# simonsobs/pixell

Measured on AMD Instinct MI355X. Metric: map2alm+alm2map round-trips/sec, higher is better.
Workload: dtype f64

## Files before the change

pixell_amd/csrc/leg_s0.hip:

```cpp
#include "legendre_dev.hpp"

namespace pxs {

#define S0_PHASE_A \
	while (k + 4 <= nk) { \
		bool act = false; \
		_Pragma("unroll") for (int s = 0; s < K; s++) act |= LEG_IS_LIVE(lam2[s], sc[s]); \
		if (__any(act)) break; \
		const double4_t q0 = LDC(coef, k), q1 = LDC(coef, k+1), q2 = LDC(coef, k+2), q3 = LDC(coef, k+3); \
		const double b0 = polar ? q0.c : q0.b, b1 = polar ? q1.c : q1.b, b2 = polar ? q2.c : q2.b, b3 = polar ? q3.c : q3.b; \
		_Pragma("unroll") for (int s = 0; s < K; s++) { \
			lam1[s] = fma(fma(q0.a, csq[s], b0), lam2[s], lam1[s]); \
			lam2[s] = fma(fma(q1.a, csq[s], b1), lam1[s], lam2[s]); \
			lam1[s] = fma(fma(q2.a, csq[s], b2), lam2[s], lam1[s]); \
			lam2[s] = fma(fma(q3.a, csq[s], b3), lam1[s], lam2[s]); \
			if (sc[s] < 0 && fabs(lam2[s]) > SC_BIG) { lam1[s] *= SC_SMALL; lam2[s] *= SC_SMALL; sc[s]++; } \
		} \
		k += 4; \
	}
#define S0_SEEDED_PHASE_A \
	if (a.seed_mode == 2) { \
		const double* sd = a.seed_d + ((long)m*a.nwave + wv)*(2*K*64); const int* si = a.seed_i + ((long)m*a.nwave + wv)*((K+1)*64); \
		k = PXS_UNIFORM_INT(si[K*64]); \
		_Pragma("unroll") for (int s = 0; s < K; s++) { lam1[s] = sd[s*64 + lane]; lam2[s] = sd[(K+s)*64 + lane]; sc[s] = si[s*64 + lane]; } \
	} else { \
		S0_PHASE_A \
		if (a.seed_mode == 1) { \
			double* sd = a.seed_d + ((long)m*a.nwave + wv)*(2*K*64); int* si = a.seed_i + ((long)m*a.nwave + wv)*((K+1)*64); \
			_Pragma("unroll") for (int s = 0; s < K; s++) { sd[s*64 + lane] = lam1[s]; sd[(K+s)*64 + lane] = lam2[s]; si[s*64 + lane] = sc[s]; } \
			if (lane == 0) si[K*64] = k; \
		} \
	}

#define S0_SYN_PAIR(c0, c1, a0, a1) { \
	PXS_VCOPY(vb0, polar ? c0.c : c0.b); \
	PXS_VCOPY(vb1, polar ? c1.c : c1.b); \
	_Pragma("unroll") for (int s = 0; s < K; s++) { \
		p1r[s] = fma(lam2[s], a0.a, p1r[s]); p1i[s] = fma(lam2[s], a0.b, p1i[s]); \
		p2r[s] = fma(lam2[s], a0.c, p2r[s]); p2i[s] = fma(lam2[s], a0.d, p2i[s]); \
		lam1[s] = fma(fma(c0.a, csq[s], vb0), lam2[s], lam1[s]); \
	} \
	_Pragma("unroll") for (int s = 0; s < K; s++) { \
		p1r[s] = fma(lam1[s], a1.a, p1r[s]); p1i[s] = fma(lam1[s], a1.b, p1i[s]); \
		p2r[s] = fma(lam1[s], a1.c, p2r[s]); p2i[s] = fma(lam1[s], a1.d, p2i[s]); \
		lam2[s] = fma(fma(c1.a, csq[s], vb1), lam1[s], lam2[s]); \
	} }

template<int K> __global__ __launch_bounds__(64, (K == 4 ? 7 : 1)) void leg_syn_s0(const LegK a)
{
	const int lane = threadIdx.x; int wv, m, bb;
	if (!leg_block(a, wv, m, bb)) return;
	const long row0 = PXS_UNIFORM_LONG(a.row[m]);
	const int nk = (a.lmax - m)/2 + 1;
	const double4_t* __restrict__ coef = a.coef + row0;
	const double4_t* __restrict__ at = reinterpret_cast<const double4_t*>(a.almt + (long)bb*a.almt_bs) + row0;
	double x[K], csq[K], lam1[K], lam2[K], p1r[K], p1i[K], p2r[K], p2i[K];
	int sc[K], rn[K], rs[K];
	bool alive_any = false;
	const bool polar = leg_wave_polar(a, wv, K);
#pragma unroll
	for (int s = 0; s < K; s++) {
		const int p = leg_pair_u(a, wv, K, s, lane);
		const bool valid = leg_pair_valid(a, p);
		rn[s] = valid ? a.ring_n[p] : -1; rs[s] = valid ? a.ring_s[p] : -1;
		x[s] = valid ? a.cth[p] : 0.0;
		const double sth = valid ? a.sth[p] : 0.0;
		csq[s] = polar ? -sth*sth : x[s]*x[s];
		const bool alive = valid && ((double)m <= a.lmax*sth + a.ofs);
		lam1[s] = 0; lam2[s] = 0; sc[s] = 0;
		if (alive && a.seed_mode != 2) { double mt; int e; pow_scaled(sth, m, mt, e); to_scaled(mt, e, lam2[s], sc[s]); }
		p1r[s] = p1i[s] = p2r[s] = p2i[s] = 0;
		alive_any |= alive;
	}
	int k = 0;
	if (__any(alive_any)) {
		S0_SEEDED_PHASE_A
		k = PXS_UNIFORM_INT(k); coef = (const double4_t*)PXS_UNIFORM_LONG((long)coef);
		PXS_COUNT(0, (long)(nk - k)*K*6 + (a.seed_mode != 2 ? (long)k*K*2 : 0L));
		while (k + 1 < nk) {
			bool pend = false;
#pragma unroll
			for (int s = 0; s < K; s++) pend |= (sc[s] < 0);
			if (!__any(pend)) break;
			for (int it = 0; it < 2 && k + 1 < nk; it++, k += 2) {
				const double4_t c0 = LDC(coef, k), c1 = LDC(coef, k+1), a0 = LDC(at, k), a1 = LDC(at, k+1);
				S0_SYN_PAIR(c0, c1, a0, a1)
			}
#pragma unroll
			for (int s = 0; s < K; s++)
				if (sc[s] < 0 && fabs(lam2[s]) > SC_BIG) {
					lam1[s] *= SC_SMALL; lam2[s] *= SC_SMALL;
					if (++sc[s] == 0) p1r[s] = p1i[s] = p2r[s] = p2i[s] = 0;
				}
		}
#pragma unroll
		for (int s = 0; s < K; s++) if (sc[s] < 0) { p1r[s] = p1i[s] = p2r[s] = p2i[s] = 0; lam1[s] = lam2[s] = 0; }
		double4_t c0 = LDC(coef, k), c1 = LDC(coef, k+1), a0 = LDC(at, k), a1 = LDC(at, k+1);
		while (k + 3 < nk) {
			double4_t n0 = LDC(coef, k+2), n1 = LDC(coef, k+3), m0 = LDC(at, k+2), m1 = LDC(at, k+3);
			S0_SYN_PAIR(c0, c1, a0, a1)
			k += 2;
			c0 = LDC(coef, k+2); c1 = LDC(coef, k+3); a0 = LDC(at, k+2); a1 = LDC(at, k+3);
			S0_SYN_PAIR(n0, n1, m0, m1)
			k += 2;
		}
		for (; k + 1 < nk; k += 2) {
			const double4_t n0 = LDC(coef, k+2), n1 = LDC(coef, k+3), m0 = LDC(at, k+2), m1 = LDC(at, k+3);
			S0_SYN_PAIR(c0, c1, a0, a1)
			c0 = n0; c1 = n1; a0 = m0; a1 = m1;
		}
		if (k < nk) {
#pragma unroll
			for (int s = 0; s < K; s++) {
				p1r[s] = fma(lam2[s], a0.a, p1r[s]); p1i[s] = fma(lam2[s], a0.b, p1i[s]);
				p2r[s] = fma(lam2[s], a0.c, p2r[s]); p2i[s] = fma(lam2[s], a0.d, p2i[s]);
			}
		}
	}
	double2* __restrict__ out = a.leg + (long)bb*a.leg_bs + (long)m*a.ld;
#pragma unroll
	for (int s = 0; s < K; s++) {
		const int p = leg_pair_u(a, wv, K, s, lane);
		const bool valid = leg_pair_valid(a, p);
		const int rn_ = valid ? a.ring_n[p] : -1, rs_ = valid ? a.ring_s[p] : -1;
		const double x_ = valid ? a.cth[p] : 0.0;
		if (rn_ >= 0) out[rn_] = make_double2(p1r[s] + x_*p2r[s], p1i[s] + x_*p2i[s]);
		if (rs_ >= 0) out[rs_] = make_double2(p1r[s] - x_*p2r[s], p1i[s] - x_*p2i[s]);
	}
}

#define S0_ANA_PAIR(c0, c1) { \
	PXS_VCOPY(vb0, polar ? c0.c : c0.b); \
	PXS_VCOPY(vb1, polar ? c1.c : c1.b); \
	double t0 = 0, t1 = 0, t2 = 0, t3 = 0, u0 = 0, u1 = 0, u2 = 0, u3 = 0; \
	_Pragma("unroll") for (int s = 0; s < K; s++) { \
		t0 = fma(lam2[s], d1r[s], t0); t1 = fma(lam2[s], d1i[s], t1); t2 = fma(lam2[s], d2r[s], t2); t3 = fma(lam2[s], d2i[s], t3); \
		lam1[s] = fma(fma(c0.a, csq[s], vb0), lam2[s], lam1[s]); \
	} \
	_Pragma("unroll") for (int s = 0; s < K; s++) { \
		u0 = fma(lam1[s], d1r[s], u0); u1 = fma(lam1[s], d1i[s], u1); u2 = fma(lam1[s], d2r[s], u2); u3 = fma(lam1[s], d2i[s], u3); \
		lam2[s] = fma(fma(c1.a, csq[s], vb1), lam1[s], lam2[s]); \
	} \
	 \
	LEG_RED_PUT(kk, t0, t1, t2, t3) \
	LEG_RED_PUT(kk+1, u0, u1, u2, u3) \
	kk += 2; \
	if (kk == LEG_FSTEPS) { leg_flush(red, pout + 4*kbase, lane, LEG_FSTEPS, a.atomic); kk = 0; kbase = k+2; } }

template<int K> __global__ __launch_bounds__(64) void leg_ana_s0(const LegK a)
{
	PXS_SHARED(double, red);
	const int lane = threadIdx.x; int wv, m, bb;
	if (!leg_block(a, wv, m, bb)) return;
	const long row0 = PXS_UNIFORM_LONG(a.row[m]);
	const int nk = (a.lmax - m)/2 + 1;
	const double4_t* __restrict__ coef = a.coef + row0;
	double* __restrict__ pout = a.part + (long)bb*a.mom_bs + ((long)wv*a.rows_chunk + (row0 - a.rowbase))*4;
	const double2* __restrict__ in = a.leg + (long)bb*a.leg_bs + (long)m*a.ld;
	double csq[K], lam1[K], lam2[K], d1r[K], d1i[K], d2r[K], d2i[K];
	int sc[K];
	bool alive_any = false;
	const bool polar = leg_wave_polar(a, wv, K);
	auto load_data = [&](int s) {
// ... 163 lines not shown
```

pixell_amd/csrc/legendre.hip:

```cpp
#include "legendre_dev.hpp"
#include <thread>
#include <memory>
#include <functional>
#include <string>

namespace pxs {

static constexpr int K_SYN0 = 4, K_ANA0 = 8, K_SYNS = 3, K_ANAS = 4;

__device__ __forceinline__ double2 ld_alm(const void* alm, int dtype, long idx) {
	if (dtype == PX_C64) { float2 v = ((const float2*)alm)[idx]; return make_double2(v.x, v.y); }
	return ((const double2*)alm)[idx];
}
__device__ __forceinline__ void st_alm(void* alm, int dtype, long idx, double2 v) {
	if (dtype == PX_C64) ((float2*)alm)[idx] = make_float2((float)v.x, (float)v.y);
	else ((double2*)alm)[idx] = v;
}
__device__ __forceinline__ double eps_lm(int l, int m) {
	if (l <= m) return 0.0;
	double L = l, M = m;
	return sqrt((L*L - M*M)/(4.0*L*L - 1.0));
}

struct AlmK {
// ... 95 lines not shown
		o[2] = -sg*be[u]*(e.x + b.y); o[3] = -sg*be[u]*(e.y - b.x);
	}
}
__global__ __launch_bounds__(256) void alm_post_spin(AlmK a) {
	const int m = blockIdx.y;
	const int l0 = max(m, a.spin);
	const int lb = blockIdx.x*(256*ALM_U) + threadIdx.x + min(m, l0);
	if (lb > a.lmax) return;
	const long base = (long)a.mstart[m], row = a.row[m];
	void* alm = alm_of_batch(a);
	double M0[ALM_U], M1[ALM_U], M2[ALM_U], M3[ALM_U], be[ALM_U];
#pragma unroll
	for (int u = 0; u < ALM_U; u++) {
		const int l = lb + 256*u;
		const bool ok = l <= a.lmax && l >= l0;
		const long r = row + (l - l0);
		const double* M = a.mom + (long)blockIdx.z*a.mom_bs + 4*r;
		M0[u] = ok ? M[0] : 0.0; M1[u] = ok ? M[1] : 0.0; M2[u] = ok ? M[2] : 0.0; M3[u] = ok ? M[3] : 0.0;
		be[u] = ok ? a.alpha[r] : 0.0;
	}
	const double sg = (a.spin & 1) ? -1.0 : 1.0;
#pragma unroll
	for (int u = 0; u < ALM_U; u++) {
		const int l = lb + 256*u;
		if (l > a.lmax) break;
		const long idx = base + (long)l*a.lstride;
		const double2 E = make_double2(-0.5*be[u]*(M0[u] + sg*M2[u]), -0.5*be[u]*(M1[u] + sg*M3[u]));
		const double2 B = make_double2(-0.5*be[u]*(M1[u] - sg*M3[u]),  0.5*be[u]*(M0[u] - sg*M2[u]));
		if (a.deriv1) { const double f = sqrt((double)l*(l+1.0)); st_alm(alm, a.dtype, idx, make_double2(f*E.x, f*E.y)); }
		else { st_alm(alm, a.dtype, idx, E); st_alm(alm, a.dtype, idx + a.cstride, B); }
	}
}

__global__ __launch_bounds__(256) void reduce_partials(const double* __restrict__ part, double* __restrict__ mom, const long* __restrict__ row,
		const int* __restrict__ first, int m0, int nmc, long rowbase, long rows_chunk, int nwave)
{
	const int mi = blockIdx.y;
	const long r0 = row[m0 + mi], nrow = row[m0 + mi + 1] - r0;
	const long i = (long)blockIdx.x*blockDim.x + threadIdx.x;
	if (i >= 4*nrow) return;
	const int step = (int)(i >> 2);
	const long off = (r0 - rowbase)*4 + i;
	double s = 0;
	for (int w = 0; w < nwave; w++) {
		const int f = first[w*nmc + mi];
		if (f > 0 && step >= f - 1) s += part[(long)w*rows_chunk*4 + off];
	}
	mom[r0*4 + i] = s;
}

__global__ __launch_bounds__(256) void coef2_kernel(const double4_t* __restrict__ coef, long nrows, double2* __restrict__ c2, double2* __restrict__ c2p) {
	const long i = (long)blockIdx.x*blockDim.x + threadIdx.x;
	if (i >= nrows + 32) return;
	if (i < nrows) { const double4_t c = coef[i]; c2[i] = make_double2(c.a, c.b); c2p[i] = make_double2(c.a, c.c); }
	else { c2[i] = make_double2(0, 0); c2p[i] = make_double2(0, 0); }
}


void LegProfile::begin(hipStream_t st, int stage) {
	if (!enabled) return;
	hipEvent_t e; PXS_HIP(hipEventCreate(&e)); PXS_HIP(hipEventRecord(e, st)); open_.push_back(e);
}
void LegProfile::end(hipStream_t st, int stage) {
	if (!enabled || open_.empty()) return;
	hipEvent_t e; PXS_HIP(hipEventCreate(&e)); PXS_HIP(hipEventRecord(e, st));
	recs.push_back(Rec{open_.back(), e, stage}); open_.pop_back();
}
void LegProfile::read(double* ms, int* counts, int nstage, bool reset) {
	for (int i = 0; i < nstage; i++) { ms[i] = 0; counts[i] = 0; }
	for (auto& r : recs) {
		PXS_HIP(hipEventSynchronize(r.b));
		float t = 0; PXS_HIP(hipEventElapsedTime(&t, r.a, r.b));
		if (r.stage >= 0 && r.stage < nstage) { ms[r.stage] += t; counts[r.stage]++; }
	}
	if (reset) { for (auto& r : recs) { (void)hipEventDestroy(r.a); (void)hipEventDestroy(r.b); } recs.clear(); }
}
LegProfile::~LegProfile() { for (auto& r : recs) { (void)hipEventDestroy(r.a); (void)hipEventDestroy(r.b); } for (auto e : open_) (void)hipEventDestroy(e); }

void RingSet::build(const std::vector<long double>& theta) {
	const long double PIl = 3.141592653589793238462643383279502884L;
	nring = (int)theta.size();
	std::vector<char> used(nring, 0);
	ring_n.clear(); ring_s.clear(); cth.clear(); sth.clear(); sh2.clear(); ch2.clear();
	std::vector<int> order(nring);
	for (int i = 0; i < nring; i++) order[i] = i;
	std::stable_sort(order.begin(), order.end(), [&](int x, int y) {
		long double a = std::min(theta[x], PIl - theta[x]), b = std::min(theta[y], PIl - theta[y]); return a < b; });
	for (int oi = 0; oi < nring; oi++) {
		int i = order[oi];
		if (used[i]) continue;
		used[i] = 1;
		int partner = -1;
		int cand = nring-1-i;
		const long double tol = 1e-12L;
		if (cand != i && cand >= 0 && !used[cand] && fabsl(theta[cand] - (PIl - theta[i])) < tol) partner = cand;
		else {
			for (int j = 0; j < nring; j++) if (!used[j] && j != i && fabsl(theta[j] - (PIl - theta[i])) < tol) { partner = j; break; }
		}
		int in_ = i, is_ = partner;
		if (partner >= 0) { used[partner] = 1; if (theta[partner] < theta[i]) { in_ = partner; is_ = i; } }
		long double th = theta[in_];
		bool flipped = false;
		if (partner < 0 && th > PIl/2) { th = PIl - th; flipped = true; }
		if (flipped) { ring_n.push_back(-1); ring_s.push_back(in_); }
		else { ring_n.push_back(in_); ring_s.push_back(is_); }
		cth.push_back((double)cosl(th)); sth.push_back((double)sinl(th));
		sh2.push_back((double)sinl(th/2)); ch2.push_back((double)cosl(th/2));
	}
// ... 27 lines not shown
	};
	if (spin == 0) {
		std::vector<LDb> cms(mmax+1);
		{ LDb cm = 1/sqrtl(4*PIl); for (int m = 0; m <= mmax; m++) { if (m > 0) cm = -cm*sqrtl((LDb)(2*m+1)/(LDb)(2*m)); cms[m] = cm; } }
		run_threads([&](int m) {
			const LDb cm = cms[m];
			auto eps = [&](int l) -> LDb { if (l <= m) return 0; LDb L = l, M = m; return sqrtl((L*L-M*M)/(4*L*L-1)); };
			const int nk = (lmax - m)/2 + 1;
			LDb a_prev = 0, a_cur = sqrtl((LDb)(2*m+3))*cm;
			for (int k = 0; k < nk; k++) {
				const int lp = m + 2*k + 1;
				const LDb e2 = eps(lp+1)*eps(lp+1) + eps(lp)*eps(lp), f = eps(lp)*eps(lp-1), d = eps(lp+1)*eps(lp+2);
				const LDb a_next = (k == 0) ? a_cur/d : -f*a_prev/d;
				const LDb ak = a_cur/(a_next*d);
				coef[row[m]+k] = double4_t{(double)ak, (double)(-ak*e2), (double)(ak - ak*e2), 0.0};
				alpha[row[m]+k] = (double)a_cur;
				a_prev = a_cur; a_cur = a_next;
			}
		});
	} else {
		const int s = spin;
		std::vector<LDb> nrm(mmax+1);
		{
			LDb h = 2*s+1; for (int i = 1; i <= s; i++) h = h*(LDb)(s+i)/(LDb)i;
			for (int m = 0; m < std::min(s, mmax+1); m++) { if (m > 0) h = h*(LDb)(s-m+1)/(LDb)(s+m); nrm[m] = sqrtl(h/(4*PIl)); }
			if (s <= mmax) {
				LDb c2 = (LDb)(2*s+1)/(4*PIl*powl(4.0L, s));
				nrm[s] = sqrtl(c2);
				for (int m = s+1; m <= mmax; m++) { c2 = c2*(LDb)(2*m+1)*(LDb)(2*m)/(4*(LDb)(m+s)*(LDb)(m-s)); nrm[m] = sqrtl(c2); }
			}
		}
		run_threads([&](int m) {
			const int l0 = std::max(m, s);
			const int nl = lmax - l0 + 1;
			if (nl <= 0) return;
			auto Sf = [&](int l) -> LDb { LDb L = l, M = m, Sp = s; return sqrtl((L*L-M*M)*(L*L-Sp*Sp)); };
			LDb b_prev = 0, b_cur = ((m & 1) ? -1 : 1)*nrm[m];
			for (int l = l0; l <= lmax; l++) {
				const LDb L = l;
				const LDb q = sqrtl((2*L+3)/(2*L+1))*(2*L+1);
				const LDb A = q*(L+1)/Sf(l+1);
				const LDb B = q*(LDb)m*(LDb)s/(L*Sf(l+1));
				const LDb C = (l > l0) ? sqrtl((2*L+3)/(2*L-1))*(L+1)*Sf(l)/(L*Sf(l+1)) : 0;
				const LDb b_next = (l == l0) ? A*b_cur : C*b_prev;
				{ const LDb ca = A*b_cur/b_next, cb = B*b_cur/b_next; coef[row[m]+(l-l0)] = double4_t{(double)ca, (double)cb, (double)(ca+cb), (double)(ca-cb)}; }
				alpha[row[m]+(l-l0)] = (double)b_cur;
				b_prev = b_cur; b_cur = b_next;
			}
		});
	}
	d_row = upload(row);
	d_coef.alloc(sizeof(double4_t)*(size_t)(nrows + 4)); PXS_HIP(hipMemcpy(d_coef.p, coef, d_coef.bytes, hipMemcpyHostToDevice));
	d_alpha.alloc(sizeof(double)*(size_t)(nrows + 4)); PXS_HIP(hipMemcpy(d_alpha.p, alpha, d_alpha.bytes, hipMemcpyHostToDevice));
}


#if defined(__clang__)
#define PXS_FP_STRICT _Pragma("clang fp contract(off)")
#else
#define PXS_FP_STRICT
#endif
struct dd { double h, l; };
__host__ __device__ __forceinline__ dd dd_norm(double a, double b) {
	PXS_FP_STRICT const double s = a + b; return dd{s, b - (s - a)}; }
__host__ __device__ __forceinline__ dd dd_of(double a) {
	PXS_FP_STRICT return dd{a, 0.0}; }
__host__ __device__ __forceinline__ dd dd_add(dd a, dd b) {
	PXS_FP_STRICT
	const double s = a.h + b.h, v = s - a.h, e = (a.h - (s - v)) + (b.h - v);
	return dd_norm(s, e + (a.l + b.l));
}
__host__ __device__ __forceinline__ dd dd_neg(dd a) {
	PXS_FP_STRICT return dd{-a.h, -a.l}; }
__host__ __device__ __forceinline__ dd dd_mul(dd a, dd b) {
	PXS_FP_STRICT
	const double p = a.h*b.h, e = fma(a.h, b.h, -p);
	return dd_norm(p, e + (a.h*b.l + a.l*b.h));
}
__host__ __device__ __forceinline__ dd dd_div(dd a, dd b) {
	PXS_FP_STRICT
	const double q1 = a.h/b.h;
	dd r = dd_add(a, dd_neg(dd_mul(dd_of(q1), b)));
	const double q2 = r.h/b.h;
	r = dd_add(r, dd_neg(dd_mul(dd_of(q2), b)));
	const double q3 = r.h/b.h;
	return dd_add(dd_norm(q1, q2), dd_of(q3));
}
__host__ __device__ __forceinline__ dd dd_sqrt(dd a) {
	PXS_FP_STRICT
	if (a.h <= 0.0) return dd{0.0, 0.0};
	const double x = sqrt(a.h);
	const double p = x*x, e = fma(x, x, -p);
	const dd r = dd_add(a, dd{-p, -e});
	return dd_norm(x, r.h/(2.0*x));
}
__host__ __device__ __forceinline__ double dd_val(dd a) {
	PXS_FP_STRICT return a.h + a.l; }

__global__ __launch_bounds__(64) void leg_tables_s0(int lmax, int mmax, const long* __restrict__ row, const dd* __restrict__ cms, double4_t* __restrict__ coef, double* __restrict__ alpha) {
	const int m = blockIdx.x*blockDim.x + threadIdx.x;
	if (m > mmax) return;
	auto q = [&](int l) -> dd { if (l <= m) return dd{0.0, 0.0}; const double L = l, M = m; return dd_div(dd_of(L*L - M*M), dd_of(4.0*L*L - 1.0)); };
	const int nk = (lmax - m)/2 + 1;
	dd a_prev = dd{0.0, 0.0}, a_cur = dd_mul(dd_sqrt(dd_of(2.0*m + 3.0)), cms[m]);
	dd qm1 = q(m), q0 = q(m + 1), qp1 = q(m + 2), qp2 = q(m + 3);
	const long r0 = row[m];
// ... 21 lines not shown
	for (int l = l0; l <= lmax; l++) {
		const double L = l;
		const dd sf1 = Sf(l + 1);
		const dd qq = dd_mul(dd_sqrt(dd_div(dd_of(2*L + 3), dd_of(2*L + 1))), dd_of(2*L + 1));
		const dd A = dd_div(dd_mul(qq, dd_of(L + 1)), sf1);
		const dd B = dd_div(dd_mul(qq, dd_of((double)m*(double)s)), dd_mul(dd_of(L), sf1));
		dd b_next;
		if (l == l0) b_next = dd_mul(A, b_cur);
		else {
			const dd C = dd_div(dd_mul(dd_mul(dd_sqrt(dd_div(dd_of(2*L + 3), dd_of(2*L - 1))), dd_of(L + 1)), sf), dd_mul(dd_of(L), sf1));
			b_next = dd_mul(C, b_prev);
		}
		const dd ca = dd_div(dd_mul(A, b_cur), b_next), cb = dd_div(dd_mul(B, b_cur), b_next);
		coef[r0 + (l - l0)] = double4_t{dd_val(ca), dd_val(cb), dd_val(dd_add(ca, cb)), dd_val(dd_add(ca, dd_neg(cb)))};
		alpha[r0 + (l - l0)] = dd_val(b_cur);
		b_prev = b_cur; b_cur = b_next; sf = sf1;
	}
}

void LegTables::build(int lmax_, int mmax_, int spin_) {
	{ const char* e = getenv("PXS_TABLES_HOST"); if (e && atoi(e) != 0) { build_host(lmax_, mmax_, spin_); return; } }
	lmax = lmax_; mmax = mmax_; spin = spin_;
	row.assign(mmax+2, 0);
	for (int m = 0; m <= mmax; m++) {
		long n = spin == 0 ? (lmax - m)/2 + 1 : std::max(0, lmax - std::max(m, spin) + 1);
		row[m+1] = row[m] + n;
	}
	nrows = row[mmax+1];
	typedef long double LDb;
	const LDb PIl = 3.141592653589793238462643383279502884L;
	std::vector<dd> start(mmax+1);
	auto put = [&](int m, LDb v) { const double h = (double)v; start[m] = dd{h, (double)(v - (LDb)h)}; };
	if (spin == 0) {
		LDb cm = 1/sqrtl(4*PIl);
		for (int m = 0; m <= mmax; m++) { if (m > 0) cm = -cm*sqrtl((LDb)(2*m+1)/(LDb)(2*m)); put(m, cm); }
	} else {
		const int s = spin;
		LDb h = 2*s+1; for (int i = 1; i <= s; i++) h = h*(LDb)(s+i)/(LDb)i;
		for (int m = 0; m < std::min(s, mmax+1); m++) { if (m > 0) h = h*(LDb)(s-m+1)/(LDb)(s+m); put(m, sqrtl(h/(4*PIl))); }
		if (s <= mmax) {
			LDb c2 = (LDb)(2*s+1)/(4*PIl*powl(4.0L, s));
			put(s, sqrtl(c2));
			for (int m = s+1; m <= mmax; m++) { c2 = c2*(LDb)(2*m+1)*(LDb)(2*m)/(4*(LDb)(m+s)*(LDb)(m-s)); put(m, sqrtl(c2)); }
		}
	}
	d_row = upload(row);
	DevBuf d_start = upload(start);
	d_coef.alloc(sizeof(double4_t)*(size_t)(nrows + 4)); d_alpha.alloc(sizeof(double)*(size_t)(nrows + 4));
	PXS_HIP(hipMemset((char*)d_coef.p + sizeof(double4_t)*(size_t)nrows, 0, sizeof(double4_t)*4)); PXS_HIP(hipMemset((char*)d_alpha.p + sizeof(double)*(size_t)nrows, 0, sizeof(double)*4));
	const dim3 grid((unsigned)((mmax + 1 + 63)/64));
	if (spin == 0) hipLaunchKernelGGL(leg_tables_s0, grid, dim3(64), 0, (hipStream_t)0, lmax, mmax, d_row.as<long>(), d_start.as<dd>(), d_coef.as<double4_t>(), d_alpha.as<double>());
	else           hipLaunchKernelGGL(leg_tables_spin, grid, dim3(64), 0, (hipStream_t)0, lmax, mmax, spin, d_row.as<long>(), d_start.as<dd>(), d_coef.as<double4_t>(), d_alpha.as<double>());
	PXS_HIP(hipGetLastError());
	PXS_HIP(hipDeviceSynchronize());
}

static long leg_almt_stride(const LegTables& tb) { return 4*(tb.nrows + 4); }
static long leg_mom_stride(const LegTables& tb) { return 4*std::max<long>(tb.nrows, 1); }
static LegK make_legk(const RingSet& rs, const LegTables& tb, LegWork& wk, double2* leg, long ld, int pairs, int nb, long leg_bs) {
	LegK a; memset(&a, 0, sizeof(a));
	a.lmax = tb.lmax; a.mmax = tb.mmax; a.spin = tb.spin; a.nm = tb.mmax+1; a.npairs = rs.npairs; a.nring = rs.nring;
	a.nwave = (rs.npairs + pairs - 1)/pairs;
	a.nrows = tb.nrows; a.row = tb.d_row.as<long>(); a.coef = tb.d_coef.as<double4_t>(); a.alpha = tb.d_alpha.as<double>();
	a.ring_n = rs.d_ring_n.as<int>(); a.ring_s = rs.d_ring_s.as<int>(); a.cth = rs.d_cth.as<double>(); a.sth = rs.d_sth.as<double>();
	a.sh2 = rs.d_sh2.as<double>(); a.ch2 = rs.d_ch2.as<double>();
	a.almt = wk.almt.as<double>(); a.part = wk.part.as<double>(); a.mom = wk.mom.as<double>();
	a.leg = leg; a.ld = ld > 0 ? ld : rs.nring;
	a.ofs = std::max(100.0, 0.01*tb.lmax);
	a.nmc = a.nm; a.xcd = 1;
	a.count = wk.count_on ? wk.count.as<double>() : nullptr;
	a.nb = nb; a.leg_bs = leg_bs; a.almt_bs = leg_almt_stride(tb); a.mom_bs = leg_mom_stride(tb);
	PXS_REQUIRE((long)8*((a.nm + 7)/8)*leg_blocks_per_m(a.nwave, nb) < (1L << 31), "internal: Legendre grid too large for one launch");
	return a;
}
static LegK make_legk_mm(const RingSet& rs, const LegTables& tb, LegWork& wk, double2* leg, long ld, int pairs, int nmaps, int ng, long leg_bs) {
	LegK a = make_legk(rs, tb, wk, leg, ld, pairs, (nmaps + 4*ng - 1)/(4*ng), leg_bs);
	a.nmaps = nmaps; a.coef2 = tb.d_coef2.as<double2>(); a.coef2p = tb.d_coef2p.as<double2>();
	return a;
}

static int leg_max_batch(const RingSet& rs, const LegTables& tb, int pairs, int cap) {
	const long nwave = (rs.npairs + (long)pairs - 1)/pairs, per_m = ((1L << 31) - 1)/(8L*((tb.mmax + 1 + 7)/8));
	const long grid = std::max<long>(1, std::min<long>(1 << 20, (per_m - 1)/std::max<long>(nwave, 1)));
	return (int)(cap > 0 ? std::min<long>(grid, cap) : grid);
}
static LegWork::Seeds* seeds_for(LegWork& wk, const RingSet& rs, const LegTables& tb, int dir, int K, LegK& a) {
	a.seed_mode = 0; a.seed_d = nullptr; a.seed_i = nullptr;
	env_budget("PXS_SEED_GB", 30, wk.seed_budget);
	if (wk.seed_budget == 0) return nullptr;
	{	const char* e = getenv("PXS_SEED_MIN_LMAX");
		const int lmin = e ? atoi(e) : (tb.spin == 0 ? 6000 : 3000);
		if (tb.lmax < lmin) return nullptr; }
	LegWork::Seeds& sb = wk.seeds[std::make_tuple((const void*)&rs, tb.spin, dir, K)];
	if (sb.refused) return nullptr;
	const int nd = tb.spin == 0 ? 2 : 4, ni = tb.spin == 0 ? 1 : 2;
	const size_t slots = (size_t)a.nm*a.nwave;
	if (!sb.d.p) {
		const size_t bd = sizeof(double)*slots*nd*K*64, bi = sizeof(int)*slots*(ni*K + 1)*64;
		if (wk.seed_bytes + bd + bi > wk.seed_budget) { sb.refused = true; return nullptr; }
		sb.d.alloc(bd); sb.i.alloc(bi); wk.seed_bytes += bd + bi;
	}
	a.seed_d = sb.d.as<double>(); a.seed_i = sb.i.as<int>(); a.seed_mode = sb.ready ? 2 : 1;
	return &sb;
}
static void seeds_written(LegWork::Seeds* sb, hipStream_t st) {
	if (!sb || sb->ready) return;
	if (!sb->written) PXS_HIP(hipEventCreateWithFlags(&sb->written, hipEventDisableTiming));
	PXS_HIP(hipEventRecord(sb->written, st)); sb->wstream = st; sb->ready = true;
}
static void seeds_wait(LegWork::Seeds* sb, hipStream_t st) {
	if (sb && sb->ready && sb->written && st != sb->wstream) PXS_HIP(hipStreamWaitEvent(st, sb->written, 0));
}

static bool seeds_pending(LegWork& wk, const RingSet& rs, const LegTables& tb, int dir, int K) {
	LegK probe; memset(&probe, 0, sizeof(probe)); probe.nm = tb.mmax + 1; probe.nwave = (rs.npairs + 64*K - 1)/(64*K);
	LegWork::Seeds* sb = seeds_for(wk, rs, tb, dir, K, probe);
	return sb != nullptr && !sb->ready;
}

static AlmK make_almk(const LegTables& tb, LegWork& wk, const void* alm, int dtype, long cstride, const uint64_t* d_mstart, long lstride, int deriv1, long alm_bs) {
	AlmK k; memset(&k, 0, sizeof(k));
	k.alm_bs = alm_bs; k.almt_bs = leg_almt_stride(tb); k.mom_bs = leg_mom_stride(tb);
	k.lmax = tb.lmax; k.mmax = tb.mmax; k.spin = tb.spin; k.deriv1 = deriv1; k.dtype = dtype;
	k.nrows = tb.nrows; k.cstride = cstride; k.lstride = lstride; k.row = tb.d_row.as<long>(); k.alpha = tb.d_alpha.as<double>();
	k.mstart = d_mstart; k.alm = const_cast<void*>(alm); k.almt = wk.almt.as<double>(); k.mom = wk.mom.as<double>();
	return k;
}

static void ensure_coef2(hipStream_t st, const LegTables& tb) {
	if (tb.d_coef2.p) return;
	tb.d_coef2.alloc(sizeof(double2)*(size_t)(tb.nrows + 32)); tb.d_coef2p.alloc(sizeof(double2)*(size_t)(tb.nrows + 32));
	hipLaunchKernelGGL(coef2_kernel, dim3((unsigned)((tb.nrows + 32 + 255)/256)), dim3(256), 0, st, tb.d_coef.as<double4_t>(), tb.nrows, tb.d_coef2.as<double2>(), tb.d_coef2p.as<double2>());
	PXS_HIP(hipStreamSynchronize(st));
}
static int k_small_grid(const RingSet& rs, int kdef, std::initializer_list<int> smaller, int kmid = 0) {
#ifdef PXS_HOST_SIM
	const bool off = [] { const char* e = getenv("PXS_K_SMALL_OFF"); return e && atoi(e) != 0; }();
#else
	constexpr bool off = false;
#endif
	if (off || rs.npairs <= 0) return kdef;
	if (rs.npairs <= 512) { int k = kdef; for (int c : smaller) k = std::min(k, c); return k; }
	if (kmid > 0 && rs.npairs <= 1400) return kmid;
	auto eligible = [&](int k) { const int last = leg_wave_last_pair(rs.npairs, k, 0); return last >= 0 && rs.cth[last]*rs.cth[last] > PXS_POLAR_COS2; };
	if (eligible(kdef)) return kdef;
	for (int k : smaller) if (k < kdef && eligible(k)) return k;
	return kdef;
}
enum LegForm { LEG_VALU, LEG_MM8, LEG_MM4 };
struct LegLaunch { int b0, n; LegForm form; int ng; };
static int mm_min(const char* name) { const char* e = getenv(name); const int x = e ? atoi(e) : 4; return x <= 0 ? (1 << 30) : std::max(2, x); }
static int syn_mm_min() { return mm_min("PXS_SYN_MM_MIN"); }
static int ana_mm_min() { return mm_min("PXS_ANA_MM_MIN"); }
static std::vector<LegLaunch> leg_batch_plan(int nb, int spin, bool analysis, int deriv1, bool deterministic, const std::function<bool()>& seeds_pending, int max_valu, int max_mm8) {
	const bool ordered = analysis && deterministic;
	const bool mm = nb >= (analysis ? ana_mm_min() : syn_mm_min()) && !ordered && !(analysis && spin > 0 && deriv1);
	std::vector<LegLaunch> plan;
	int b = 0;
	if (mm) {
		const int nmm = nb - (nb % 8 == 1 ? 1 : 0), r = nmm % 8, n8 = nmm - r;
		for (; b < n8; b += max_mm8) plan.push_back({b, std::min(max_mm8, n8 - b), LEG_MM8, 2});
		if (r > 4) plan.push_back({n8, r, LEG_MM8, 2}); else if (r > 0) plan.push_back({n8, r, LEG_MM4, 1});
		b = nmm;
	}
	if (ordered || (nb - b > 1 && seeds_pending())) for (const int e = ordered ? nb : b + 1; b < e; b++) plan.push_back({b, 1, LEG_VALU, 0});
	for (; b < nb; b += max_valu) plan.push_back({b, std::min(max_valu, nb - b), LEG_VALU, 0});
	return plan;
}
static void print_batch_plan(bool analysis, int spin, int nb, const std::vector<LegLaunch>& plan) {
	if (!getenv("PXS_CHAIN_VERBOSE")) return;
	std::string s;
	for (const LegLaunch& l : plan) s += std::string(l.form == LEG_VALU ? " VALU [" : l.form == LEG_MM8 ? " mm8 [" : " mm4 [") + std::to_string(l.b0) + "," + std::to_string(l.b0 + l.n) + ")";
	fprintf(stderr, "[pxsht] legendre %s spin %d, %d maps:%s\n", analysis ? "analysis" : "synthesis", spin, nb, s.c_str());
}

void leg_synthesis(hipStream_t st, const RingSet& rs, const LegTables& tb, LegWork& wk,
                   const void* alm, int alm_dtype, long alm_cstride, const uint64_t* d_mstart, long lstride,
                   double2* leg, int deriv1, LegProfile* prof, long ld, int nb, long alm_bstride, long leg_bstride)
{
	PXS_REQUIRE(alm_dtype == PX_C64 || alm_dtype == PX_C128, "alm must be complex64 or complex128");
	PXS_REQUIRE(nb >= 1, "leg_synthesis: nb must be >= 1");
	wk.almt.ensure(sizeof(double)*(size_t)leg_almt_stride(tb)*nb);
	AlmK ak = make_almk(tb, wk, alm, alm_dtype, alm_cstride, d_mstart, lstride, deriv1, alm_bstride);
	const int nm = tb.mmax+1;
	const int K = tb.spin == 0 ? k_small_grid(rs, K_SYN0, {2}, 2) : k_small_grid(rs, K_SYNS, {2}, 2);
	const int mm_pairs = tb.spin == 0 ? 64 : 32;
	if (tb.spin == 0) hipLaunchKernelGGL(alm_pre_s0, alm_grid(tb.lmax/2 + 1, nm, nb), dim3(256), 0, st, ak);
	else              hipLaunchKernelGGL(alm_pre_spin, alm_grid(tb.lmax + 1, nm, nb), dim3(256), 0, st, ak);
	const std::vector<LegLaunch> plan = leg_batch_plan(nb, tb.spin, false, deriv1, wk.deterministic, [&] { return seeds_pending(wk, rs, tb, 0, K); },
		leg_max_batch(rs, tb, 64*K, wk.max_batch), 8*leg_max_batch(rs, tb, mm_pairs, wk.max_batch));
	print_batch_plan(false, tb.spin, nb, plan);
	wk.pass_valu.begin(); wk.pass_mm.begin();
	for (const LegLaunch& l : plan) {
		(l.ng ? wk.pass_mm : wk.pass_valu).add(l.n);
		double2* legl = leg + (size_t)l.b0*leg_bstride;
		if (l.ng) ensure_coef2(st, tb);
		LegK a = l.ng ? make_legk_mm(rs, tb, wk, legl, ld, mm_pairs, l.n, l.ng, leg_bstride) : make_legk(rs, tb, wk, legl, ld, 64*K, l.n, leg_bstride);
		a.almt += (size_t)l.b0*a.almt_bs;
		LegWork::Seeds* sb = nullptr;
		if (!l.ng) { sb = seeds_for(wk, rs, tb, 0, K, a); seeds_wait(sb, st); }
		if (prof) prof->begin(st, 0);
		(tb.spin == 0 ? launch_leg_s0 : launch_leg_spin)(false, l.ng, K, leg_grid(a), st, a);
		if (prof) prof->end(st, 0);
		seeds_written(sb, st);
	}
	PXS_HIP(hipGetLastError());
}

static void leg_analysis_valu(hipStream_t st, const RingSet& rs, const LegTables& tb, LegWork& wk, int K, const double2* leg, double* mom, LegProfile* prof, long ld, int nb, long leg_bstride)
{
	const int nm = tb.mmax+1, nwave = (rs.npairs + 64*K - 1)/(64*K);
	const bool atomic = !wk.deterministic;
	std::vector<int> cuts; cuts.push_back(0);
	if (atomic) cuts.push_back(nm);
	else {
		const size_t budget = wk.part_budget;
		for (int m = 0; m < nm;) {
			int m1 = m+1;
			while (m1 < nm && (size_t)(tb.row[m1+1]-tb.row[m])*32*nwave <= budget) m1++;
			cuts.push_back(m1); m = m1;
		}
		size_t maxrows = 1;
		for (size_t c = 0; c+1 < cuts.size(); c++) maxrows = std::max<size_t>(maxrows, (size_t)(tb.row[cuts[c+1]]-tb.row[cuts[c]]));
		wk.part.ensure(sizeof(double)*4*maxrows*nwave);
		size_t maxm = 1;
		for (size_t c = 0; c+1 < cuts.size(); c++) maxm = std::max<size_t>(maxm, (size_t)(cuts[c+1]-cuts[c]));
		wk.first.ensure(sizeof(int)*(size_t)nwave*maxm);
	}
	LegWork::Seeds* seeds = nullptr;
	wk.pass_m.begin();
	for (size_t c = 0; c+1 < cuts.size(); c++) {
		const int m0 = cuts[c], m1 = cuts[c+1];
		const long rows = tb.row[m1]-tb.row[m0];
		if (rows <= 0) continue;
		wk.pass_m.add(m1 - m0);
		LegK a = make_legk(rs, tb, wk, const_cast<double2*>(leg), ld, 64*K, nb, leg_bstride);
		a.mom = mom; a.m0 = m0; a.rowbase = tb.row[m0]; a.rows_chunk = rows; a.nmc = m1-m0; a.atomic = atomic ? 1 : 0;
		seeds = seeds_for(wk, rs, tb, 1, K, a); seeds_wait(seeds, st);
		if (atomic) { a.part = mom; a.rowbase = 0; a.rows_chunk = 0; a.first = nullptr; }
		else {
			PXS_HIP(hipMemsetAsync(wk.first.p, 0, sizeof(int)*(size_t)nwave*(m1-m0), st));
			a.first = wk.first.as<int>();
		}
		if (prof) prof->begin(st, 1);
		const dim3 grid = leg_grid(a);
		(tb.spin == 0 ? launch_leg_s0 : launch_leg_spin)(true, 0, K, grid, st, a);
		if (prof) prof->end(st, 1);
		if (atomic) continue;
		const long maxrow = tb.row[m0+1] - tb.row[m0];
		hipLaunchKernelGGL(reduce_partials, dim3((unsigned)((4*maxrow+255)/256), m1-m0), dim3(256), 0, st, (const double*)wk.part.p,
			mom, tb.d_row.as<long>(), (const int*)wk.first.p, m0, m1-m0, tb.row[m0], rows, a.nwave);
	}
	seeds_written(seeds, st);
}

void leg_analysis(hipStream_t st, const RingSet& rs, const LegTables& tb, LegWork& wk,
                  const double2* leg, void* alm, int alm_dtype, long alm_cstride, const uint64_t* d_mstart, long lstride,
                  int deriv1, LegProfile* prof, long ld, int nb, long alm_bstride, long leg_bstride)
{
	PXS_REQUIRE(alm_dtype == PX_C64 || alm_dtype == PX_C128, "alm must be complex64 or complex128");
	PXS_REQUIRE(nb >= 1, "leg_analysis: nb must be >= 1");
	const int K = tb.spin == 0 ? k_small_grid(rs, K_ANA0, {4, 2}, 4) : k_small_grid(rs, K_ANAS, {3, 2});
	const int nm = tb.mmax+1;
	const int mm_pairs = (tb.spin == 0 ? 64 : 32)*MM_WAVES;
	const std::vector<LegLaunch> plan = leg_batch_plan(nb, tb.spin, true, deriv1, wk.deterministic, [&] { return seeds_pending(wk, rs, tb, 1, K); },
		leg_max_batch(rs, tb, 64*K, wk.max_batch), 8*leg_max_batch(rs, tb, mm_pairs, wk.max_batch));
	print_batch_plan(true, tb.spin, nb, plan);
	const size_t nmom = (size_t)leg_mom_stride(tb);
	wk.mom.ensure(sizeof(double)*nmom*nb);
	if (!wk.deterministic) PXS_HIP(hipMemsetAsync(wk.mom.p, 0, sizeof(double)*nmom*nb, st));
	wk.pass_valu.begin(); wk.pass_mm.begin();
	for (const LegLaunch& l : plan) {
		(l.ng ? wk.pass_mm : wk.pass_valu).add(l.n);
		const double2* legl = leg + (size_t)l.b0*leg_bstride;
		double* mom = wk.mom.as<double>() + nmom*l.b0;
		if (!l.ng) { leg_analysis_valu(st, rs, tb, wk, K, legl, mom, prof, ld, l.n, leg_bstride); continue; }
		ensure_coef2(st, tb);
		LegK a = make_legk_mm(rs, tb, wk, const_cast<double2*>(legl), ld, mm_pairs, l.n, l.ng, leg_bstride);
		a.mom = mom; a.part = mom; a.atomic = 1;
		if (prof) prof->begin(st, 1);
		(tb.spin == 0 ? launch_leg_s0 : launch_leg_spin)(true, l.ng, K, leg_grid(a), st, a);
		if (prof) prof->end(st, 1);
	}
	AlmK ak = make_almk(tb, wk, alm, alm_dtype, alm_cstride, d_mstart, lstride, deriv1, alm_bstride);
	if (tb.spin == 0) hipLaunchKernelGGL(alm_post_s0, alm_grid(tb.lmax/2 + 1, nm, nb), dim3(256), 0, st, ak);
	else              hipLaunchKernelGGL(alm_post_spin, alm_grid(tb.lmax + 1, nm, nb), dim3(256), 0, st, ak);
	PXS_HIP(hipGetLastError());
}

}
```

pixell_amd/csrc/legendre.hpp:

```cpp
#pragma once
#include <map>
#include <tuple>
#include "common.hpp"

namespace pxs {

struct RingSet {
	int nring = 0;
	int npairs = 0;
	std::vector<int> ring_n, ring_s;
	std::vector<double> cth, sth, sh2, ch2;
	DevBuf d_ring_n, d_ring_s, d_cth, d_sth, d_sh2, d_ch2;
	void build(const std::vector<long double>& theta);
	void upload_all();
};

struct LegTables {
	int lmax = 0, mmax = 0, spin = 0;
	std::vector<long> row;
	long nrows = 0;
	DevBuf d_row, d_coef, d_alpha;
	mutable DevBuf d_coef2, d_coef2p;
	void build(int lmax, int mmax, int spin);
	void build_host(int lmax, int mmax, int spin);
};

struct LegProfile {
	struct Rec { hipEvent_t a, b; int stage; };
	std::vector<Rec> recs; std::vector<hipEvent_t> open_;
	bool enabled = false;
	void begin(hipStream_t st, int stage);
	void end(hipStream_t st, int stage);
	void read(double* ms, int* counts, int nstage, bool reset);
	~LegProfile();
};

struct LegWork {
	size_t part_budget = size_t(2) << 30;
	bool deterministic = false;
	DevBuf almt;
	DevBuf part;
	DevBuf mom;
	DevBuf first;
	struct Seeds { DevBuf d, i; bool ready = false, refused = false; hipEvent_t written = nullptr; hipStream_t wstream = nullptr;
	               ~Seeds() { if (written) (void)hipEventDestroy(written); } };
	std::map<std::tuple<const void*, int, int, int>, Seeds> seeds;
	size_t seed_budget = size_t(16) << 30, seed_bytes = 0;
	DevBuf count; bool count_on = false;
	int max_batch = 0;
	PassLog pass_m, pass_valu, pass_mm;
};


void leg_synthesis(hipStream_t st, const RingSet& rs, const LegTables& tb, LegWork& wk,
                   const void* alm, int alm_dtype, long alm_cstride, const uint64_t* d_mstart, long lstride,
                   double2* leg, int deriv1, LegProfile* prof = nullptr, long ld = 0, int nb = 1, long alm_bstride = 0, long leg_bstride = 0);
void leg_analysis(hipStream_t st, const RingSet& rs, const LegTables& tb, LegWork& wk,
                  const double2* leg, void* alm, int alm_dtype, long alm_cstride, const uint64_t* d_mstart, long lstride,
                  int deriv1, LegProfile* prof = nullptr, long ld = 0, int nb = 1, long alm_bstride = 0, long leg_bstride = 0);

}
```

pixell_amd/csrc/legendre_dev.hpp:

```cpp
#pragma once
#include "legendre.hpp"
#include <cmath>
#include <algorithm>
#include <initializer_list>

namespace pxs {

static constexpr double SC_BIG   = 0x1p+400;
static constexpr double SC_SMALL = 0x1p-800;
static constexpr int    SC_STEP  = 800;
static constexpr double LEG_LIVE = 0x1p-140;
#define LEG_IS_LIVE(v, sc) ((sc) == 0 && fabs(v) >= LEG_LIVE)

struct double4_t { double a, b, c, d; };
#ifdef PXS_HOST_SIM
#define LDC(p, i) ((p)[i])
#else
typedef double pxs_d4 __attribute__((ext_vector_type(4)));
__device__ __forceinline__ double4_t ldc_row(const double4_t* p, long i) {
	const __attribute__((address_space(4))) pxs_d4* c = (const __attribute__((address_space(4))) pxs_d4*)(unsigned long long)p;
	const pxs_d4 v = c[i]; double4_t r; r.a = v.x; r.b = v.y; r.c = v.z; r.d = v.w; return r;
}
#define LDC(p, i) ldc_row((p), (i))
#endif
#ifdef PXS_HOST_SIM
#define LDCD(p, i) ((p)[i])
#else
__device__ __forceinline__ double ldc_double(const double* p, long i) {
	const __attribute__((address_space(4))) double* c = (const __attribute__((address_space(4))) double*)(unsigned long long)p;
	return c[i];
}
#define LDCD(p, i) ldc_double((p), (i))
#endif

struct LegK {
	int lmax, mmax, spin, nm, npairs, nring, nwave;
	long ld;
	long nrows;
	const long* row; const double4_t* coef; const double* alpha;
	const int* ring_n; const int* ring_s; const double* cth; const double* sth; const double* sh2; const double* ch2;
	double* almt; double* part; double* mom;
	double2* leg;
	double ofs;
	int m0; long rowbase, rows_chunk;
	int nmc, xcd;
	int* first;
	int atomic;
	int seed_mode; double* seed_d; int* seed_i;
	double* count;
	int nb; long leg_bs, almt_bs, mom_bs;
	int nmaps;
	const double2* coef2; const double2* coef2p;
};
#define PXS_NCOUNT 1024
#ifdef PXS_HOST_SIM
#define PXS_COUNT(dir, expr) if (a.count != nullptr && lane == 0) atomicAdd(a.count + 2*(blockIdx.x & (PXS_NCOUNT - 1)) + (dir), (double)(expr))
#else
#define PXS_COUNT(dir, expr) if (a.count != nullptr && lane == 0) unsafeAtomicAdd(a.count + 2*(blockIdx.x & (PXS_NCOUNT - 1)) + (dir), (double)(expr))
#endif

__host__ __device__ constexpr unsigned leg_blocks_per_m(unsigned nwave, unsigned nb) { return (nwave*nb) | 1u; }
static_assert(leg_blocks_per_m(20, 1) == 21 && leg_blocks_per_m(27, 1) == 27 && leg_blocks_per_m(4, 8) == 33 && leg_blocks_per_m(3, 2) == 7, "blocks per m: odd, at most one more than chunks x maps");
__device__ __forceinline__ bool leg_block(const LegK& a, int& wv, int& m, int& bb) {
	if (!a.xcd) { wv = blockIdx.x; m = blockIdx.y + a.m0; bb = blockIdx.z; return true; }
	const unsigned b = blockIdx.x, x = b & 7u, j = b >> 3;
	const unsigned per_m = leg_blocks_per_m((unsigned)a.nwave, (unsigned)a.nb);
	const unsigned ml = j / per_m, r = j - ml*per_m;
	bb = (int)(r / (unsigned)a.nwave);
	wv = (int)(r - (unsigned)bb*a.nwave);
	const unsigned mi = ml*8u + x;
	m = (int)mi + a.m0;
	return mi < (unsigned)a.nmc && bb < a.nb;
}
static inline dim3 leg_grid(const LegK& a) { return a.xcd ? dim3((unsigned)(8*((a.nmc+7)/8)*leg_blocks_per_m(a.nwave, a.nb))) : dim3(a.nwave, a.nmc, a.nb); }

__device__ __forceinline__ void frexp_norm(double& m, int& e) { int d; m = frexp(m, &d); e += d; }

__device__ __forceinline__ void pow_scaled(double x, int n, double& mant, int& e) {
	double rm = 0.5; int re = 1;
	int be = 0; double bm = frexp(x, &be);
	while (n) {
		if (n & 1) { rm *= bm; re += be; frexp_norm(rm, re); }
		bm *= bm; be *= 2; frexp_norm(bm, be);
		n >>= 1;
	}
// ... 391 lines not shown
```

Before: 3.590.

## Use compact two-double coefficient rows in spin-0 synthesis steady-state loop

The spin-0 synthesis main loop now reads precomputed compact coefficient arrays (a plus b, or a plus c for polar waves) as one 32-byte scalar load per pair of rows, instead of two 32-byte double4 rows. The compact tables are now built eagerly at table construction for all paths rather than lazily for the matrix path only. Explicit scalar-memory waitcnt drains and scheduling barriers are added to control load issue and overlap with the FMA work. This halves the scalar coefficient traffic, but the forced waits and sched barriers may restrict compiler scheduling and add extra table memory.

```diff
diff --git a/pixell_amd/csrc/leg_s0.hip b/pixell_amd/csrc/leg_s0.hip
--- a/pixell_amd/csrc/leg_s0.hip
+++ b/pixell_amd/csrc/leg_s0.hip
@@ -32,18 +32,19 @@
 		} \
 	}
 
-#define S0_SYN_PAIR(c0, c1, a0, a1) { \
-	PXS_VCOPY(vb0, polar ? c0.c : c0.b); \
-	PXS_VCOPY(vb1, polar ? c1.c : c1.b); \
+#define S0_SYN_PAIR(c0, c1, a0, a1) S0_SYN_PAIR_C(c0.a, polar ? c0.c : c0.b, c1.a, polar ? c1.c : c1.b, a0, a1)
+#define S0_SYN_PAIR_C(ca0, cb0, ca1, cb1, a0, a1) { \
+	PXS_VCOPY(vb0, cb0); \
+	PXS_VCOPY(vb1, cb1); \
 	_Pragma("unroll") for (int s = 0; s < K; s++) { \
 		p1r[s] = fma(lam2[s], a0.a, p1r[s]); p1i[s] = fma(lam2[s], a0.b, p1i[s]); \
 		p2r[s] = fma(lam2[s], a0.c, p2r[s]); p2i[s] = fma(lam2[s], a0.d, p2i[s]); \
-		lam1[s] = fma(fma(c0.a, csq[s], vb0), lam2[s], lam1[s]); \
+		lam1[s] = fma(fma(ca0, csq[s], vb0), lam2[s], lam1[s]); \
 	} \
 	_Pragma("unroll") for (int s = 0; s < K; s++) { \
 		p1r[s] = fma(lam1[s], a1.a, p1r[s]); p1i[s] = fma(lam1[s], a1.b, p1i[s]); \
 		p2r[s] = fma(lam1[s], a1.c, p2r[s]); p2i[s] = fma(lam1[s], a1.d, p2i[s]); \
-		lam2[s] = fma(fma(c1.a, csq[s], vb1), lam1[s], lam2[s]); \
+		lam2[s] = fma(fma(ca1, csq[s], vb1), lam1[s], lam2[s]); \
 	} }
 
 template<int K> __global__ __launch_bounds__(64, (K == 4 ? 7 : 1)) void leg_syn_s0(const LegK a)
@@ -95,20 +96,27 @@
 		}
 #pragma unroll
 		for (int s = 0; s < K; s++) if (sc[s] < 0) { p1r[s] = p1i[s] = p2r[s] = p2i[s] = 0; lam1[s] = lam2[s] = 0; }
-		double4_t c0 = LDC(coef, k), c1 = LDC(coef, k+1), a0 = LDC(at, k), a1 = LDC(at, k+1);
+		const double2* __restrict__ cf = (const double2*)PXS_UNIFORM_LONG((long)((polar ? a.coef2p : a.coef2) + row0));
+		coef2x2_t f = LDC2(cf, k); double4_t a0 = LDC(at, k), a1 = LDC(at, k+1);
 		while (k + 3 < nk) {
-			double4_t n0 = LDC(coef, k+2), n1 = LDC(coef, k+3), m0 = LDC(at, k+2), m1 = LDC(at, k+3);
-			S0_SYN_PAIR(c0, c1, a0, a1)
-			k += 2;
-			c0 = LDC(coef, k+2); c1 = LDC(coef, k+3); a0 = LDC(at, k+2); a1 = LDC(at, k+3);
-			S0_SYN_PAIR(n0, n1, m0, m1)
-			k += 2;
+			PXS_ROWS_DRAIN();
+			coef2x2_t n = LDC2(cf, k+2); double4_t m0 = LDC(at, k+2), m1 = LDC(at, k+3);
+			PXS_ROWS_ISSUED();
+			S0_SYN_PAIR_C(f.a0, f.b0, f.a1, f.b1, a0, a1)
+			PXS_ROWS_DRAIN();
+			f = LDC2(cf, k+4); a0 = LDC(at, k+4); a1 = LDC(at, k+5);
+			PXS_ROWS_ISSUED();
+			S0_SYN_PAIR_C(n.a0, n.b0, n.a1, n.b1, m0, m1)
+			k += 4;
 		}
 		for (; k + 1 < nk; k += 2) {
-			const double4_t n0 = LDC(coef, k+2), n1 = LDC(coef, k+3), m0 = LDC(at, k+2), m1 = LDC(at, k+3);
-			S0_SYN_PAIR(c0, c1, a0, a1)
-			c0 = n0; c1 = n1; a0 = m0; a1 = m1;
-		}
+			PXS_ROWS_DRAIN();
+			const coef2x2_t n = LDC2(cf, k+2); const double4_t m0 = LDC(at, k+2), m1 = LDC(at, k+3);
+			PXS_ROWS_ISSUED();
+			S0_SYN_PAIR_C(f.a0, f.b0, f.a1, f.b1, a0, a1)
+			f = n; a0 = m0; a1 = m1;
+		}
+		PXS_ROWS_DRAIN();
 		if (k < nk) {
 #pragma unroll
 			for (int s = 0; s < K; s++) {
diff --git a/pixell_amd/csrc/legendre.hip b/pixell_amd/csrc/legendre.hip
--- a/pixell_amd/csrc/legendre.hip
+++ b/pixell_amd/csrc/legendre.hip
@@ -171,8 +171,9 @@
 __global__ __launch_bounds__(256) void coef2_kernel(const double4_t* __restrict__ coef, long nrows, double2* __restrict__ c2, double2* __restrict__ c2p) {
 	const long i = (long)blockIdx.x*blockDim.x + threadIdx.x;
 	if (i >= nrows + 32) return;
-	if (i < nrows) { const double4_t c = coef[i]; c2[i] = make_double2(c.a, c.b); c2p[i] = make_double2(c.a, c.c); }
-	else { c2[i] = make_double2(0, 0); c2p[i] = make_double2(0, 0); }
+	const double4_t c = i < nrows ? coef[i] : double4_t{0, 0, 0, 0};
+	c2[i] = make_double2(c.a, c.b);
+	if (c2p) c2p[i] = make_double2(c.a, c.c);
 }
 
 
@@ -306,6 +307,7 @@
 	d_row = upload(row);
 	d_coef.alloc(sizeof(double4_t)*(size_t)(nrows + 4)); PXS_HIP(hipMemcpy(d_coef.p, coef, d_coef.bytes, hipMemcpyHostToDevice));
 	d_alpha.alloc(sizeof(double)*(size_t)(nrows + 4)); PXS_HIP(hipMemcpy(d_alpha.p, alpha, d_alpha.bytes, hipMemcpyHostToDevice));
+	build_compact();
 }
 
 
@@ -433,6 +435,14 @@
 	if (spin == 0) hipLaunchKernelGGL(leg_tables_s0, grid, dim3(64), 0, (hipStream_t)0, lmax, mmax, d_row.as<long>(), d_start.as<dd>(), d_coef.as<double4_t>(), d_alpha.as<double>());
 	else           hipLaunchKernelGGL(leg_tables_spin, grid, dim3(64), 0, (hipStream_t)0, lmax, mmax, spin, d_row.as<long>(), d_start.as<dd>(), d_coef.as<double4_t>(), d_alpha.as<double>());
 	PXS_HIP(hipGetLastError());
+	build_compact();
+}
+
+void LegTables::build_compact() {
+	d_coef2.alloc(sizeof(double2)*(size_t)(nrows + 32));
+	if (spin == 0) d_coef2p.alloc(sizeof(double2)*(size_t)(nrows + 32));
+	hipLaunchKernelGGL(coef2_kernel, dim3((unsigned)((nrows + 32 + 255)/256)), dim3(256), 0, (hipStream_t)0, d_coef.as<double4_t>(), nrows, d_coef2.as<double2>(), d_coef2p.as<double2>());
+	PXS_HIP(hipGetLastError());
 	PXS_HIP(hipDeviceSynchronize());
 }
 
@@ -450,13 +460,14 @@
 	a.ofs = std::max(100.0, 0.01*tb.lmax);
 	a.nmc = a.nm; a.xcd = 1;
 	a.count = wk.count_on ? wk.count.as<double>() : nullptr;
+	a.coef2 = tb.d_coef2.as<double2>(); a.coef2p = tb.d_coef2p.as<double2>();
 	a.nb = nb; a.leg_bs = leg_bs; a.almt_bs = leg_almt_stride(tb); a.mom_bs = leg_mom_stride(tb);
 	PXS_REQUIRE((long)8*((a.nm + 7)/8)*leg_blocks_per_m(a.nwave, nb) < (1L << 31), "internal: Legendre grid too large for one launch");
 	return a;
 }
 static LegK make_legk_mm(const RingSet& rs, const LegTables& tb, LegWork& wk, double2* leg, long ld, int pairs, int nmaps, int ng, long leg_bs) {
 	LegK a = make_legk(rs, tb, wk, leg, ld, pairs, (nmaps + 4*ng - 1)/(4*ng), leg_bs);
-	a.nmaps = nmaps; a.coef2 = tb.d_coef2.as<double2>(); a.coef2p = tb.d_coef2p.as<double2>();
+	a.nmaps = nmaps;
 	return a;
 }
 
@@ -508,12 +519,6 @@
 	return k;
 }
 
-static void ensure_coef2(hipStream_t st, const LegTables& tb) {
-	if (tb.d_coef2.p) return;
-	tb.d_coef2.alloc(sizeof(double2)*(size_t)(tb.nrows + 32)); tb.d_coef2p.alloc(sizeof(double2)*(size_t)(tb.nrows + 32));
-	hipLaunchKernelGGL(coef2_kernel, dim3((unsigned)((tb.nrows + 32 + 255)/256)), dim3(256), 0, st, tb.d_coef.as<double4_t>(), tb.nrows, tb.d_coef2.as<double2>(), tb.d_coef2p.as<double2>());
-	PXS_HIP(hipStreamSynchronize(st));
-}
 static int k_small_grid(const RingSet& rs, int kdef, std::initializer_list<int> smaller, int kmid = 0) {
 #ifdef PXS_HOST_SIM
 	const bool off = [] { const char* e = getenv("PXS_K_SMALL_OFF"); return e && atoi(e) != 0; }();
@@ -575,7 +580,6 @@
 	for (const LegLaunch& l : plan) {
 		(l.ng ? wk.pass_mm : wk.pass_valu).add(l.n);
 		double2* legl = leg + (size_t)l.b0*leg_bstride;
-		if (l.ng) ensure_coef2(st, tb);
 		LegK a = l.ng ? make_legk_mm(rs, tb, wk, legl, ld, mm_pairs, l.n, l.ng, leg_bstride) : make_legk(rs, tb, wk, legl, ld, 64*K, l.n, leg_bstride);
 		a.almt += (size_t)l.b0*a.almt_bs;
 		LegWork::Seeds* sb = nullptr;
@@ -656,7 +660,6 @@
 		const double2* legl = leg + (size_t)l.b0*leg_bstride;
 		double* mom = wk.mom.as<double>() + nmom*l.b0;
 		if (!l.ng) { leg_analysis_valu(st, rs, tb, wk, K, legl, mom, prof, ld, l.n, leg_bstride); continue; }
-		ensure_coef2(st, tb);
 		LegK a = make_legk_mm(rs, tb, wk, const_cast<double2*>(legl), ld, mm_pairs, l.n, l.ng, leg_bstride);
 		a.mom = mom; a.part = mom; a.atomic = 1;
 		if (prof) prof->begin(st, 1);
diff --git a/pixell_amd/csrc/legendre.hpp b/pixell_amd/csrc/legendre.hpp
--- a/pixell_amd/csrc/legendre.hpp
+++ b/pixell_amd/csrc/legendre.hpp
@@ -20,7 +20,8 @@
 	std::vector<long> row;
 	long nrows = 0;
 	DevBuf d_row, d_coef, d_alpha;
-	mutable DevBuf d_coef2, d_coef2p;
+	DevBuf d_coef2, d_coef2p;
+	void build_compact();
 	void build(int lmax, int mmax, int spin);
 	void build_host(int lmax, int mmax, int spin);
 };
diff --git a/pixell_amd/csrc/legendre_dev.hpp b/pixell_amd/csrc/legendre_dev.hpp
--- a/pixell_amd/csrc/legendre_dev.hpp
+++ b/pixell_amd/csrc/legendre_dev.hpp
@@ -31,6 +31,22 @@
 	return c[i];
 }
 #define LDCD(p, i) ldc_double((p), (i))
+#endif
+
+struct coef2x2_t { double a0, b0, a1, b1; };
+#ifdef PXS_HOST_SIM
+#define LDC2(p, i) (coef2x2_t{(p)[i].x, (p)[i].y, (p)[(i)+1].x, (p)[(i)+1].y})
+#define PXS_ROWS_DRAIN()
+#define PXS_ROWS_ISSUED()
+#else
+typedef double pxs_d4a16 __attribute__((ext_vector_type(4), aligned(16)));
+__device__ __forceinline__ coef2x2_t ldc_row2(const double2* p, long i) {
+	const __attribute__((address_space(4))) pxs_d4a16* c = (const __attribute__((address_space(4))) pxs_d4a16*)(unsigned long long)(p + i);
+	const pxs_d4a16 v = *c; coef2x2_t r; r.a0 = v.x; r.b0 = v.y; r.a1 = v.z; r.b1 = v.w; return r;
+}
+#define LDC2(p, i) ldc_row2((p), (i))
+#define PXS_ROWS_DRAIN() do { __builtin_amdgcn_s_waitcnt(0xc07f); __builtin_amdgcn_sched_barrier(0); } while (0)
+#define PXS_ROWS_ISSUED() __builtin_amdgcn_sched_barrier(0)
 #endif
 
 struct LegK {
```

After: 3.626, median of 6. 1.01x the previous value.
